# ZhiHuangHn/vtkCloudPoint

Measured on AMD Instinct MI355X. Metric: Mpoints/s DBSCAN+label @10M pts, higher is better.
Workload: dtype f64; 1 GPU; C4: 10000000-pt cloud (half uniform background, 200 Gaussian blobs), one monolithic DBImproved.dbscan, metric L1_2D, eps 0.1, minPts 10; mode=single, points_total=10000000, points_per_gpu=10000000, clusters=27380, resident_in_hbm=True

## Files before the change

vtkcloudpoint_amd/csrc/gridbuild.hip:

```cpp
#include <algorithm>
#include <mutex>
#include <unordered_map>

#include "grid_common.hpp"

using namespace vcpg;

namespace {

constexpr int PT = 1024;
constexpr int PCH_MIN = 8192;
constexpr int FT = 1024;
constexpr uint32_t MAXB = 8192;
constexpr uint32_t wcap(int) { return 4096u; }
constexpr uint32_t QUEUE_FROM = 32;

typedef float4 Rec;

template <int GD>
__device__ __forceinline__ Rec rec_make(const float* qf, uint32_t idx, uint32_t cell) {
  return GD == 2 ? make_float4(qf[0], qf[1], __uint_as_float(idx), __uint_as_float(cell))
                 : make_float4(qf[0], qf[1], qf[2], __uint_as_float(idx));
}
template <int GD>
__device__ __forceinline__ uint32_t rec_cell(const Rec& r, const GridP& g, uint32_t& idx) {
  if (GD == 2) {
    idx = __float_as_uint(r.z);
    return __float_as_uint(r.w);
  }
  idx = __float_as_uint(r.w);
  const float qf[3] = {r.x, r.y, r.z};
  int cc[3];
  return cell_of32<3>(qf, g, cc);
}

template <int GD>
__device__ __forceinline__ uint32_t point_cell(const double* __restrict__ c, int64_t i, int stride, const GridP& g, float* qf) {
  double q[3];
  int cc[3];
  load_in<GD>(c, i, stride, q);
#pragma unroll
  for (int a = 0; a < GD; a++) qf[a] = rel32(q[a], g.mn[a], g.scale);
  return cell_of32<GD>(qf, g, cc);
}

struct PartGeom {
  uint32_t csh;
  uint32_t B;
  uint32_t a;
  uint32_t NS;
  uint32_t chunk;
  uint32_t nchunk;
};

inline int env_int(const char* name, int dflt, int lo, int hi) {
  const char* e = getenv(name);
  int v = e ? atoi(e) : dflt;
  return v < lo ? lo : v > hi ? hi : v;
}

inline PartGeom part_geom(int64_t n, uint32_t ncells) {
  static const int csh_max = env_int("VCP_CPB_LOG2", 14, 10, 14);
  static const int target = env_int("VCP_PART_CHUNKS", 256, 64, 8192);
  PartGeom p;
  int csh = csh_max;
  while (csh > 10 && ((uint64_t)ncells >> csh) * 4096ull < (uint64_t)n) csh--;
  p.csh = (uint32_t)csh;
  p.B = (uint32_t)((((uint64_t)ncells + 1) + ((1ull << p.csh) - 1)) >> p.csh);
  p.a = 0;
  while (((p.B + (1u << p.a) - 1u) >> p.a) > MAXB) p.a++;
  p.NS = (p.B + (1u << p.a) - 1u) >> p.a;
  int64_t chunk = (n + target - 1) / target;
  if (chunk < PCH_MIN) chunk = PCH_MIN;
  chunk = (chunk + PT - 1) / PT * PT;
  p.chunk = (uint32_t)chunk;
  p.nchunk = (uint32_t)((n + chunk - 1) / chunk);
  return p;
}

template <int GD, bool GROUPED>
__global__ __launch_bounds__(PT) void k_part_hist(const double* __restrict__ c, int64_t n, int stride, GridP g,
                                                 const int32_t* __restrict__ group, int glo, int ghi, uint32_t csh,
                                                 uint32_t B, uint32_t chunk, uint32_t nchunk,
                                                 uint32_t* __restrict__ counts, uint32_t* __restrict__ qcount,
                                                 uint32_t* __restrict__ ctcount) {
  extern __shared__ uint32_t h[];
  if (blockIdx.x == 0 && threadIdx.x == 0) {
    *qcount = 0u;
    ctcount[0] = 0u;
  }
  for (uint32_t k = threadIdx.x; k < B; k += PT) h[k] = 0;
  __syncthreads();
  const int64_t first = (int64_t)blockIdx.x * chunk;
  const int64_t last = min(first + (int64_t)chunk, n);
#pragma unroll 4
  for (int64_t i = first + threadIdx.x; i < last; i += PT) {
    if (GROUPED) {
      const int gg = group[i];
      if (gg < glo || gg >= ghi) continue;
    }
    float qf[3];
    atomicAdd(&h[point_cell<GD>(c, i, stride, g, qf) >> csh], 1u);
  }
  __syncthreads();
  for (uint32_t k = threadIdx.x; k < B; k += PT) counts[(size_t)k * nchunk + blockIdx.x] = h[k];
}

template <int GD, bool GROUPED>
__global__ __launch_bounds__(PT) void k_part_scatter(const double* __restrict__ c, int64_t n, int stride, GridP g,
                                                    const int32_t* __restrict__ group, int glo, int ghi, uint32_t csh,
                                                    uint32_t B, uint32_t chunk, uint32_t nchunk,
                                                    const uint32_t* __restrict__ base, Rec* __restrict__ rec,
                                                    uint32_t* __restrict__ pos) {
  extern __shared__ uint32_t h[];
  for (uint32_t k = threadIdx.x; k < B; k += PT) h[k] = base[(size_t)k * nchunk + blockIdx.x];
  __syncthreads();
  const int64_t first = (int64_t)blockIdx.x * chunk;
  const int64_t last = min(first + (int64_t)chunk, n);
#pragma unroll 4
  for (int64_t i = first + threadIdx.x; i < last; i += PT) {
    if (GROUPED) {
      const int gg = group[i];
      if (gg < glo || gg >= ghi) {
        if (pos) pos[i] = NONE;
        continue;
      }
    }
    float qf[3];
    const uint32_t cell = point_cell<GD>(c, i, stride, g, qf);
    rec[atomicAdd(&h[cell >> csh], 1u)] = rec_make<GD>(qf, (uint32_t)i, cell);
  }
}

__device__ __forceinline__ uint32_t padded(uint32_t i) { return i + (i >> 5); }

template <int GD, bool GROUPED, int NT = FT>
__device__ __forceinline__ void fine_flush(uint32_t s0, uint32_t m, const float* s32, const uint32_t* sidx,
                                           const uint32_t* __restrict__ ord, const uint8_t* __restrict__ in_classed,
                                           const int32_t* __restrict__ group, float* __restrict__ sorted32,
                                           uint32_t* __restrict__ sord, uint32_t* __restrict__ sidx_out,
                                           int32_t* __restrict__ sgroup, uint8_t* __restrict__ flags,
                                           uint32_t* __restrict__ pos) {
  if (GD == 2) {
    const float2* src = reinterpret_cast<const float2*>(s32);
    float2* dst = reinterpret_cast<float2*>(sorted32) + s0;
    for (uint32_t k = threadIdx.x; k < m; k += NT) dst[k] = src[k];
  } else {
    const float4* src = reinterpret_cast<const float4*>(s32);
    float4* dst = reinterpret_cast<float4*>(sorted32) + s0;
    for (uint32_t k = threadIdx.x; k < m; k += NT) dst[k] = src[k];
  }
  for (uint32_t k = threadIdx.x; k < m; k += NT) {
    const uint32_t i = sidx[k], p = s0 + k;
    sord[p] = ord ? ord[i] : i;
    if (sidx_out) sidx_out[p] = i;
    if (GROUPED) sgroup[p] = group[i];
    if (in_classed) flags[p] = in_classed[i] ? F_CLASSED : 0;
    if (pos) pos[i] = p;
  }
}

template <int GD>
__device__ __forceinline__ void stage_put(float* s32, uint32_t* sidx, uint32_t p, const Rec& r, uint32_t idx) {
  if (GD == 2) reinterpret_cast<float2*>(s32)[p] = make_float2(r.x, r.y);
  else reinterpret_cast<float4*>(s32)[p] = make_float4(r.x, r.y, r.z, 0.0f);
  sidx[p] = idx;
}

__device__ __forceinline__ void bucket_range(const uint32_t* __restrict__ bstart, uint32_t bstride, const uint32_t* __restrict__ total,
                                             uint32_t b, uint32_t B, uint32_t& s, uint32_t& e) {
  s = bstart[(size_t)b * bstride];
  e = (b + 1 < B) ? bstart[(size_t)(b + 1) * bstride] : *total;
}

template <int GD>
__global__ __launch_bounds__(FT) void k_part_split(const Rec* __restrict__ rec, Rec* __restrict__ rec2,
                                                  const uint32_t* __restrict__ base, const uint32_t* __restrict__ total,
                                                  uint32_t nchunk, uint32_t NS, uint32_t a, uint32_t csh, uint32_t B, GridP g,
                                                  uint32_t* __restrict__ bstart) {
  __shared__ uint32_t h[32];
  const uint32_t S = blockIdx.x;
  uint32_t s, e;
  bucket_range(base, nchunk, total, S, NS, s, e);
  const uint32_t subm = (1u << a) - 1u;
  if (threadIdx.x < 32) h[threadIdx.x] = 0u;
  __syncthreads();
  for (uint32_t j = s + threadIdx.x; j < e; j += FT) {
    uint32_t i;
    atomicAdd(&h[(rec_cell<GD>(rec[j], g, i) >> csh) & subm], 1u);
  }
  __syncthreads();
  if (threadIdx.x < 32) {
    const uint32_t v = h[threadIdx.x];
    uint32_t inc = v;
#pragma unroll
    for (int d = 1; d < 32; d <<= 1) {
      const uint32_t t = __shfl_up(inc, d, 64);
      if ((int)threadIdx.x >= d) inc += t;
    }
    const uint32_t first = s + inc - v;
    h[threadIdx.x] = first;
    const uint32_t bk = (S << a) + threadIdx.x;
    if (threadIdx.x <= subm && bk <= B) bstart[bk] = first;
  }
  __syncthreads();
  for (uint32_t j = s + threadIdx.x; j < e; j += FT) {
    const Rec r = rec[j];
    uint32_t i;
    rec2[atomicAdd(&h[(rec_cell<GD>(r, g, i) >> csh) & subm], 1u)] = r;
  }
}

constexpr int FS = 512;
constexpr uint32_t scap(int gd) { return gd == 2 ? 2048u : 1536u; }
constexpr uint32_t SPOP = 128;

template <int GD, bool GROUPED>
__global__ __launch_bounds__(FS) void k_part_fine_small(const Rec* __restrict__ rec, const uint32_t* __restrict__ bstart,
                                                       uint32_t bstride, const uint32_t* __restrict__ total, uint32_t B,
                                                       uint32_t csh, GridP g, const uint32_t* __restrict__ ord,
                                                       const uint8_t* __restrict__ in_classed, const int32_t* __restrict__ group,
                                                       uint4* __restrict__ ctwords, uint32_t* __restrict__ ctdense,
                                                       uint32_t* __restrict__ ctcount, uint8_t* __restrict__ bstate,
                                                       float* __restrict__ sorted32, uint32_t* __restrict__ sord,
                                                       uint32_t* __restrict__ sidx_out, int32_t* __restrict__ sgroup,
                                                       uint8_t* __restrict__ flags, uint32_t* __restrict__ pos) {
  constexpr uint32_t FPR = GD == 2 ? 2 : 4;
  constexpr uint32_t SCAP = scap(GD);
  constexpr int SRPT = SCAP / FS;
  __shared__ uint32_t ws[512 + 2];
  __shared__ uint32_t wlo[512], whi[512];
  __shared__ uint16_t wpi[512];
  __shared__ uint8_t sci[SCAP];
  __shared__ __attribute__((aligned(16))) uint16_t st32[SPOP][32];
  __shared__ __attribute__((aligned(16))) float s32[SCAP * FPR];
  __shared__ uint32_t sidx[SCAP];
  __shared__ uint32_t wsum[FS / 64];
  __shared__ uint32_t s_np, s_dbase;
  const uint32_t b = blockIdx.x;
  uint32_t s, e;
  bucket_range(bstart, bstride, total, b, B, s, e);
  const uint32_t m = e - s;
  if (b + 1 == B && threadIdx.x == 0) ctcount[1] = *total;
  if (m > SCAP) {
    if (threadIdx.x == 0) bstate[b] = 1;
    return;
  }
  const uint32_t CPB = 1u << csh, NW = CPB >> 5, c0 = b << csh;
  const int lane = threadIdx.x & 63, w = threadIdx.x >> 6;
  for (uint32_t k = threadIdx.x; k < NW + 1; k += FS) ws[k] = 0u;
  __syncthreads();
  Rec r[SRPT];
  uint32_t idx[SRPT], lw[SRPT], ci[SRPT], rnk[SRPT];
#pragma unroll
  for (int k = 0; k < SRPT; k++) {
    const uint32_t j = s + (uint32_t)k * FS + threadIdx.x;
    lw[k] = NONE;
    if (j < e) {
      r[k] = rec[j];
      const uint32_t c = rec_cell<GD>(r[k], g, idx[k]) - c0;
      lw[k] = c >> 5;
      ci[k] = c & 31u;
      rnk[k] = atomicAdd(&ws[lw[k]], 1u);
    }
  }
  __syncthreads();
  {
    const uint32_t v = threadIdx.x < NW ? ws[threadIdx.x] : 0u;
    uint32_t inc = v;
#pragma unroll
    for (int d = 1; d < 64; d <<= 1) {
      const uint32_t t = __shfl_up(inc, d, 64);
      if (lane >= d) inc += t;
    }
    if (lane == 63) wsum[w] = inc;
    __syncthreads();
    uint32_t pre = inc - v;
    for (int k = 0; k < w; k++) pre += wsum[k];
    if (threadIdx.x < NW) ws[threadIdx.x] = s + pre;
    if (threadIdx.x == 0) ws[NW] = e;
  }
  __syncthreads();
#pragma unroll
  for (int k = 0; k < SRPT; k++)
    if (lw[k] != NONE) sci[ws[lw[k]] - s + rnk[k]] = (uint8_t)ci[k];
  __syncthreads();
  bool popl = false;
  uint32_t lo = 0u, hi = 0u;
  if (threadIdx.x < NW) {
    const uint32_t a = ws[threadIdx.x] - s, k = ws[threadIdx.x + 1] - s - a;
    if (k > 64u) {
      popl = true;
    } else {
      for (uint32_t i = 0; i < k; i++) {
        const uint32_t bit = 1u << sci[a + i];
        if (lo & hi & bit) continue;
        if (lo & bit) hi ^= bit;
        lo ^= bit;
      }
      popl = (lo & hi) != 0u;
    }
  }
  {
    const unsigned long long dm = __ballot(popl);
    if (lane == 0) wsum[w] = (uint32_t)__popcll(dm);
    __syncthreads();
    uint32_t before = (uint32_t)__popcll(dm & ((1ull << lane) - 1ull)), tot = 0;
    for (int k = 0; k < FS / 64; k++) {
      if (k < w) before += wsum[k];
      tot += wsum[k];
    }
    if (threadIdx.x == 0) s_np = tot;
    if (threadIdx.x < NW) wpi[threadIdx.x] = popl ? (uint16_t)before : (uint16_t)0xFFFFu;
  }
  __syncthreads();
  const uint32_t np = s_np;
  if (np > SPOP) {
    if (threadIdx.x == 0) bstate[b] = 1;
    return;
  }
  if (threadIdx.x == 0) {
    bstate[b] = 0;
    s_dbase = np ? atomicAdd(&ctcount[0], np) : 0u;
  }
  for (uint32_t k = threadIdx.x; k < np * 16u; k += FS) reinterpret_cast<uint32_t*>(&st32[0][0])[k] = 0u;
  if (threadIdx.x < NW && !popl) {
    wlo[threadIdx.x] = lo;
    whi[threadIdx.x] = hi;
  }
  __syncthreads();
#pragma unroll
  for (int k = 0; k < SRPT; k++)
    if (lw[k] != NONE && wpi[lw[k]] != 0xFFFFu) {
      uint16_t* c = &st32[wpi[lw[k]]][ci[k]];
      atomicAdd(reinterpret_cast<uint32_t*>(reinterpret_cast<uintptr_t>(c) & ~(uintptr_t)3), ((uintptr_t)c & 2) ? 0x10000u : 1u);
    }
  __syncthreads();
  {
    const uint32_t hw = threadIdx.x >> 5, li = threadIdx.x & 31u;
    for (uint32_t wd = hw; wd < NW; wd += FS / 32) {
      const uint32_t pi = wpi[wd];
      if (pi == 0xFFFFu) continue;
      const uint32_t c = st32[pi][li];
      uint32_t inc = c;
#pragma unroll
      for (int d = 1; d < 32; d <<= 1) {
        const uint32_t t = __shfl_up(inc, d, 32);
        if ((int)li >= d) inc += t;
      }
      const uint32_t first = ws[wd] + inc - c;
      st32[pi][li] = (uint16_t)(first - s);
      ctdense[(size_t)(s_dbase + pi) * 32u + li] = first;
      const uint32_t cs = min(c, 3u);
      const unsigned long long blo = __ballot(cs & 1u), bhi = __ballot(cs >> 1);
      const int sh = (threadIdx.x & 32) ? 32 : 0;
      if (li == 0) {
        wlo[wd] = (uint32_t)(blo >> sh);
        whi[wd] = (uint32_t)(bhi >> sh);
      }
    }
  }
  __syncthreads();
#pragma unroll
  for (int k = 0; k < SRPT; k++) {
    if (lw[k] == NONE) continue;
    const uint32_t pi = wpi[lw[k]];
    uint32_t p;
    if (pi != 0xFFFFu) {
      uint16_t* c = &st32[pi][ci[k]];
      const bool up = ((uintptr_t)c & 2) != 0;
      const uint32_t old = atomicAdd(reinterpret_cast<uint32_t*>(reinterpret_cast<uintptr_t>(c) & ~(uintptr_t)3), up ? 0x10000u : 1u);
      p = up ? old >> 16 : old & 0xFFFFu;
    } else {
      const uint32_t l = wlo[lw[k]], h = whi[lw[k]], below = (1u << ci[k]) - 1u;
      const uint32_t a = ws[lw[k]] - s;
      p = a + (uint32_t)__popc(l & below) + 2u * (uint32_t)__popc(h & below);
      if ((h >> ci[k]) & 1u)
        for (uint32_t i = 0; i < rnk[k]; i++) p += sci[a + i] == (uint8_t)ci[k] ? 1u : 0u;
    }
    stage_put<GD>(s32, sidx, p, r[k], idx[k]);
  }
  if (threadIdx.x < NW) {
    const size_t W = (size_t)(c0 >> 5) + threadIdx.x;
    const uint32_t pi = wpi[threadIdx.x];
    if (W < vcp_ct_words(g.ncells))
      ctwords[W] = make_uint4(wlo[threadIdx.x], whi[threadIdx.x], ws[threadIdx.x], pi != 0xFFFFu ? s_dbase + pi : NONE);
  }
  __syncthreads();
  fine_flush<GD, GROUPED, FS>(s, m, s32, sidx, ord, in_classed, group, sorted32, sord, sidx_out, sgroup, flags, pos);
}

template <int GD, bool GROUPED>
__global__ __launch_bounds__(FT) void k_part_fine(const Rec* __restrict__ rec, uint32_t* __restrict__ rk,
                                                 const uint32_t* __restrict__ bstart, uint32_t bstride,
                                                 const uint32_t* __restrict__ total, uint32_t B, uint32_t csh, GridP g,
                                                 const uint32_t* __restrict__ ord, const uint8_t* __restrict__ in_classed,
                                                 const int32_t* __restrict__ group, uint4* __restrict__ ctwords,
                                                 uint32_t* __restrict__ ctdense, uint32_t* __restrict__ ctcount,
                                                 float* __restrict__ sorted32, uint32_t* __restrict__ sord,
                                                 uint32_t* __restrict__ sidx_out, int32_t* __restrict__ sgroup,
                                                 uint8_t* __restrict__ flags, uint32_t* __restrict__ pos,
                                                 uint2* __restrict__ queue, uint32_t* __restrict__ qcount,
                                                 const uint8_t* __restrict__ bstate) {
  extern __shared__ __attribute__((aligned(16))) unsigned char lds[];
  __shared__ uint32_t wsum[FT / 64];
  __shared__ uint32_t w_lo[512], w_hi[512], w_slot[512];
  __shared__ uint32_t s_dbase;
  const uint32_t b = blockIdx.x;
  if (bstate[b] == 0) return;
  constexpr uint32_t WCAP = wcap(GD);
  constexpr uint32_t FPR = GD == 2 ? 2 : 4;
  const uint32_t CPB = 1u << csh;
  uint32_t* cnt = reinterpret_cast<uint32_t*>(lds);
  float* s32 = reinterpret_cast<float*>(lds + (((size_t)padded(CPB) + 4) & ~3ull) * 4);
  uint32_t* sidx = reinterpret_cast<uint32_t*>(s32 + (size_t)WCAP * FPR);
  const uint32_t c0 = b << csh;
  uint32_t s, e;
  bucket_range(bstart, bstride, total, b, B, s, e);
  const uint32_t m = e - s;
  const bool big = m > WCAP;
  for (uint32_t k = threadIdx.x; k < padded(CPB); k += FT) cnt[k] = 0;
  __syncthreads();
  for (uint32_t j = s + threadIdx.x; j < e; j += FT) {
    uint32_t i;
    uint32_t* slot = &cnt[padded(rec_cell<GD>(rec[j], g, i) - c0)];
    if (big) rk[j] = atomicAdd(slot, 1u);
    else atomicAdd(slot, 1u);
  }
  __syncthreads();
  const uint32_t PER = CPB / FT;
  const uint32_t first = threadIdx.x * PER;
  uint32_t loc = 0;
  for (uint32_t k = 0; k < PER; k++) loc += cnt[padded(first + k)];
  const int lane = threadIdx.x & 63, w = threadIdx.x >> 6;
  uint32_t inc = loc;
#pragma unroll
  for (int d = 1; d < 64; d <<= 1) {
    const uint32_t t = __shfl_up(inc, d, 64);
    if (lane >= d) inc += t;
  }
  if (lane == 63) wsum[w] = inc;
  __syncthreads();
  uint32_t pre = s + inc - loc;
  for (int k = 0; k < w; k++) pre += wsum[k];
  const uint32_t NW = CPB >> 5;
  uint32_t plo = 0u, phi = 0u;
  const uint32_t wstart = pre;
  {
    const uint32_t bit0 = first & 31u;
    for (uint32_t k = 0; k < PER; k++) {
      const uint32_t v = cnt[padded(first + k)];
      cnt[padded(first + k)] = pre;
      pre += v;
      const uint32_t c = min(v, 3u);
      plo |= (c & 1u) << (bit0 + k);
      phi |= (c >> 1) << (bit0 + k);
    }
    for (uint32_t d = 1; d < 32u / PER; d <<= 1) {
      plo |= (uint32_t)__shfl_xor((int)plo, (int)d, 64);
      phi |= (uint32_t)__shfl_xor((int)phi, (int)d, 64);
    }
    if ((first & 31u) == 0u) {
      w_lo[first >> 5] = plo;
      w_hi[first >> 5] = phi;
      w_slot[first >> 5] = wstart;
    }
  }
  __syncthreads();
  {
    const bool popl = threadIdx.x < NW && (w_lo[threadIdx.x] & w_hi[threadIdx.x]) != 0u;
    const unsigned long long dm = __ballot(popl);
    if (lane == 0) wsum[w] = (uint32_t)__popcll(dm);
    __syncthreads();
    uint32_t before = (uint32_t)__popcll(dm & ((1ull << lane) - 1ull)), tot = 0;
    for (int k = 0; k < FT / 64; k++) {
      if (k < w) before += wsum[k];
      tot += wsum[k];
    }
    if (threadIdx.x == 0) s_dbase = tot ? atomicAdd(&ctcount[0], tot) : 0u;
    __syncthreads();
    if (threadIdx.x < NW) {
      const uint32_t slot = popl ? s_dbase + before : NONE;
      const uint32_t wpos = w_slot[threadIdx.x];
      w_slot[threadIdx.x] = slot;
      const size_t W = (size_t)(c0 >> 5) + threadIdx.x;
      if (W < vcp_ct_words(g.ncells))
        ctwords[W] = make_uint4(w_lo[threadIdx.x], w_hi[threadIdx.x], wpos, slot);
    }
    __syncthreads();
    const uint32_t hw = threadIdx.x >> 5, li = threadIdx.x & 31u;
    for (uint32_t j = hw; j < NW; j += FT / 32) {
      const uint32_t slot = w_slot[j];
      if (slot != NONE) ctdense[(size_t)slot * 32u + li] = cnt[padded(32u * j + li)];
    }
  }
  __syncthreads();
  if (!big) {
    for (uint32_t j = s + threadIdx.x; j < e; j += FT) {
      const Rec r = rec[j];
      uint32_t i;
      const uint32_t p = atomicAdd(&cnt[padded(rec_cell<GD>(r, g, i) - c0)], 1u) - s;
      stage_put<GD>(s32, sidx, p, r, i);
    }
    __syncthreads();
    fine_flush<GD, GROUPED>(s, m, s32, sidx, ord, in_classed, group, sorted32, sord, sidx_out, sgroup, flags, pos);
    return;
  }
  if (m > QUEUE_FROM * WCAP) {
    __shared__ uint32_t q0;
    const uint32_t nwin = (m + WCAP - 1) / WCAP;
    if (threadIdx.x == 0) q0 = atomicAdd(qcount, nwin);
    __syncthreads();
    for (uint32_t k = threadIdx.x; k < nwin; k += FT) queue[q0 + k] = make_uint2(b, k * WCAP);
    return;
  }
  for (uint32_t w0 = 0; w0 < m; w0 += WCAP) {
    for (uint32_t j = s + threadIdx.x; j < e; j += FT) {
      const Rec r = rec[j];
      uint32_t i;
      const uint32_t p = cnt[padded(rec_cell<GD>(r, g, i) - c0)] + rk[j] - s - w0;
      if (p < WCAP) stage_put<GD>(s32, sidx, p, r, i);
    }
    __syncthreads();
    fine_flush<GD, GROUPED>(s + w0, min(WCAP, m - w0), s32, sidx, ord, in_classed, group, sorted32, sord, sidx_out, sgroup,
                            flags, pos);
    __syncthreads();
  }
}

template <int GD, bool GROUPED>
__global__ __launch_bounds__(FT) void k_part_fine_windows(const Rec* __restrict__ rec, const uint32_t* __restrict__ rk,
                                                         const uint32_t* __restrict__ bstart, uint32_t bstride,
                                                         const uint32_t* __restrict__ total, uint32_t B, GridP g,
                                                         const uint32_t* __restrict__ ord, const uint8_t* __restrict__ in_classed,
                                                         const int32_t* __restrict__ group, CellTab ct,
                                                         float* __restrict__ sorted32,
                                                         uint32_t* __restrict__ sord, uint32_t* __restrict__ sidx_out,
                                                         int32_t* __restrict__ sgroup, uint8_t* __restrict__ flags,
                                                         uint32_t* __restrict__ pos, const uint2* __restrict__ queue,
                                                         const uint32_t* __restrict__ qcount) {
  extern __shared__ __attribute__((aligned(16))) unsigned char lds[];
  constexpr uint32_t WCAP = wcap(GD);
  constexpr uint32_t FPR = GD == 2 ? 2 : 4;
  float* s32 = reinterpret_cast<float*>(lds);
  uint32_t* sidx = reinterpret_cast<uint32_t*>(s32 + (size_t)WCAP * FPR);
  const uint32_t nq = *qcount;
  for (uint32_t qi = blockIdx.x; qi < nq; qi += gridDim.x) {
    const uint2 q = queue[qi];
    const uint32_t b = q.x, w0 = q.y;
    uint32_t s, e;
    bucket_range(bstart, bstride, total, b, B, s, e);
    const uint32_t m = e - s;
    for (uint32_t j = s + threadIdx.x; j < e; j += FT) {
      const Rec r = rec[j];
      uint32_t i;
      const uint32_t p = ct_start(ct, rec_cell<GD>(r, g, i)) + rk[j] - s - w0;
      if (p < WCAP) stage_put<GD>(s32, sidx, p, r, i);
    }
    __syncthreads();
    fine_flush<GD, GROUPED>(s + w0, min(WCAP, m - w0), s32, sidx, ord, in_classed, group, sorted32, sord, sidx_out, sgroup,
                            flags, pos);
    __syncthreads();
  }
}

constexpr int OT = 1024, OPT = 16;
constexpr int OWT = 512;

template <int OWSH>
__global__ __launch_bounds__(OT) void k_out_scatter(const uint32_t* __restrict__ sord, const uint32_t* __restrict__ labk,
                                                   int64_t n, uint32_t OB, uint32_t* __restrict__ gcur,
                                                   uint2* __restrict__ rec) {
  extern __shared__ uint32_t h[];
  for (uint32_t k = threadIdx.x; k < OB; k += OT) h[k] = 0;
  __syncthreads();
  const int64_t first = (int64_t)blockIdx.x * (OT * OPT);
  uint32_t o[OPT], w[OPT], r[OPT];
#pragma unroll
  for (int k = 0; k < OPT; k++) {
    const int64_t p = first + (int64_t)k * OT + threadIdx.x;
    o[k] = NONE;
    if (p < n) {
      o[k] = sord[p];
      w[k] = labk[p];
      r[k] = atomicAdd(&h[o[k] >> OWSH], 1u);
    }
  }
  __syncthreads();
  for (uint32_t k = threadIdx.x; k < OB; k += OT) {
    const uint32_t c = h[k];
    if (c) h[k] = atomicAdd(&gcur[k], c);
  }
  __syncthreads();
#pragma unroll
  for (int k = 0; k < OPT; k++) {
    if (o[k] == NONE) continue;
    const uint32_t bk = o[k] >> OWSH;
    rec[((size_t)bk << OWSH) + h[bk] + r[k]] = make_uint2(o[k], w[k]);
  }
}

template <int OWSH>
__global__ __launch_bounds__(OWT) void k_out_write(const uint2* __restrict__ rec, int64_t n, bool have_in_classed,
                                                  int32_t cf_in, int32_t* __restrict__ labels,
                                                  uint8_t* __restrict__ is_core, uint8_t* __restrict__ is_classed,
                                                  unsigned long long* __restrict__ counters, uint32_t* __restrict__ gcur) {
  extern __shared__ __attribute__((aligned(16))) uint32_t sw[];
  if (threadIdx.x == 0) gcur[blockIdx.x] = 0u;
  const int64_t lo = (int64_t)blockIdx.x << OWSH;
  const uint32_t cnt = (uint32_t)min((int64_t)1 << OWSH, n - lo);
  unsigned unclassed = 0;
  for (uint32_t j = threadIdx.x; j < cnt; j += OWT) {
    const uint2 v = rec[lo + j];
    sw[v.x - (uint32_t)lo] = v.y;
    if (!(v.y & 2u)) unclassed++;
  }
  __syncthreads();
  auto lab_of = [&](uint32_t w) { return (w >> 2) ? cf_in + (int32_t)(w >> 2) : 0; };
  auto core_of = [](uint32_t w) { return (uint32_t)((w & 3u) == 1u); };
  auto cls_of = [](uint32_t w) { return (uint32_t)((w & 2u) != 0u || (w >> 2) != 0u); };
  const bool vec = (((uintptr_t)labels & 15u) | ((uintptr_t)is_core & 3u) | ((uintptr_t)is_classed & 3u)) == 0;
  const uint32_t c4 = vec ? cnt >> 2 : 0u;
  for (uint32_t j = threadIdx.x; j < c4; j += OWT) {
    const uint4 w = reinterpret_cast<const uint4*>(sw)[j];
    const int4 l = make_int4(lab_of(w.x), lab_of(w.y), lab_of(w.z), lab_of(w.w));
    if (have_in_classed) {
      if (l.x) labels[lo + 4 * j] = l.x;
      if (l.y) labels[lo + 4 * j + 1] = l.y;
      if (l.z) labels[lo + 4 * j + 2] = l.z;
      if (l.w) labels[lo + 4 * j + 3] = l.w;
    } else {
      reinterpret_cast<int4*>(labels + lo)[j] = l;
    }
    if (is_core)
      reinterpret_cast<uint32_t*>(is_core + lo)[j] = core_of(w.x) | core_of(w.y) << 8 | core_of(w.z) << 16 | core_of(w.w) << 24;
    if (is_classed)
      reinterpret_cast<uint32_t*>(is_classed + lo)[j] = cls_of(w.x) | cls_of(w.y) << 8 | cls_of(w.z) << 16 | cls_of(w.w) << 24;
  }
  for (uint32_t j = (c4 << 2) + threadIdx.x; j < cnt; j += OWT) {
    const uint32_t w = sw[j];
    const int32_t l = lab_of(w);
    if (!have_in_classed || l) labels[lo + j] = l;
    if (is_core) is_core[lo + j] = (uint8_t)core_of(w);
    if (is_classed) is_classed[lo + j] = (uint8_t)cls_of(w);
  }
  if (have_in_classed) {
    __shared__ unsigned wc[OWT / 64];
#pragma unroll
    for (int d = 32; d > 0; d >>= 1) unclassed += __shfl_down(unclassed, d, 64);
    if ((threadIdx.x & 63) == 0) wc[threadIdx.x >> 6] = unclassed;
    __syncthreads();
    if (threadIdx.x == 0) {
      unsigned t = 0;
      for (int k = 0; k < OWT / 64; k++) t += wc[k];
      if (t) atomicAdd(&counters[CNT_UNCLASSED + (blockIdx.x & (CNT_SPREAD - 1))], (unsigned long long)t);
    }
  }
}

int allow_lds(vcp_ctx* ctx, const void* kernel, size_t bytes) {
  static std::mutex mu;
  static std::unordered_map<uint64_t, size_t> allowed;
  std::lock_guard<std::mutex> lk(mu);
  const uint64_t key = (uint64_t)reinterpret_cast<uintptr_t>(kernel) * 64u + (uint64_t)(ctx->device & 63);
  size_t& have = allowed.emplace(key, (size_t)64 * 1024).first->second;
  if (bytes > have) {
    VCP_HIP(ctx, hipFuncSetAttribute(kernel, hipFuncAttributeMaxDynamicSharedMemorySize, (int)bytes));
    have = bytes;
  }
  return VCP_OK;
}
template <class K>
int allow_lds(vcp_ctx* ctx, K kernel, size_t bytes) {
  return allow_lds(ctx, reinterpret_cast<const void*>(kernel), bytes);
}

template <int GD, bool GROUPED>
int build(vcp_ctx* ctx, const GridBuildArgs& a) {
  hipStream_t st = ctx->stream;
  const PartGeom pg = part_geom(a.n, a.g.ncells);
  const size_t nc = (size_t)pg.NS * pg.nchunk;
  VCP_TRY(vcp_ensure(ctx, ctx->b_hist, (nc + 8) * 4));
  VCP_TRY(vcp_ensure(ctx, ctx->b_rec, (size_t)a.n * sizeof(Rec)));
  uint32_t* counts = ctx->b_hist.as<uint32_t>();
  uint32_t* total = counts + nc;
  Rec* rec = ctx->b_rec.as<Rec>();
  const size_t lds_h = (size_t)pg.NS * 4;
  const uint32_t CPB = 1u << pg.csh;
  const size_t lds_f = ((((size_t)CPB + CPB / 32) + 4) & ~3ull) * 4 + (size_t)wcap(GD) * ((GD == 2 ? 8 : 16) + 4);
  VCP_TRY(allow_lds(ctx, k_part_fine<GD, GROUPED>, lds_f));
  VCP_TRY(vcp_ensure(ctx, ctx->b_fineq, ((size_t)a.n / wcap(GD) + pg.B + 8) * sizeof(uint2) + 64));
  uint32_t* qcount = ctx->b_fineq.as<uint32_t>();
  uint2* queue = reinterpret_cast<uint2*>(ctx->b_fineq.as<char>() + 64);
  vcp_phase(ctx, "part_hist");
  const uint32_t csh_a = pg.csh + pg.a;
  VCP_LAUNCH(ctx, (k_part_hist<GD, GROUPED>), dim3(pg.nchunk), dim3(PT), lds_h, st, a.d_coords, a.n, a.stride, a.g,
                  a.d_group, a.glo, a.ghi, csh_a, pg.NS, pg.chunk, pg.nchunk, counts, qcount, a.ctcount);
  VCP_TRY(vcp_exclusive_scan_u32(ctx, counts, counts, (int64_t)nc, total));
  vcp_phase(ctx, "part_scatter");
  VCP_LAUNCH(ctx, (k_part_scatter<GD, GROUPED>), dim3(pg.nchunk), dim3(PT), lds_h, st, a.d_coords, a.n, a.stride, a.g,
                  a.d_group, a.glo, a.ghi, csh_a, pg.NS, pg.chunk, pg.nchunk, counts, rec, a.pos);
  const uint32_t* bstart = counts;
  uint32_t bstride = pg.nchunk;
  if (pg.a > 0) {
    vcp_phase(ctx, "part_split");
    VCP_TRY(vcp_ensure(ctx, ctx->b_rec2, (size_t)a.n * sizeof(Rec)));
    VCP_TRY(vcp_ensure(ctx, ctx->b_bstart, ((size_t)pg.B + 2) * 4));
    VCP_LAUNCH(ctx, k_part_split<GD>, dim3(pg.NS), dim3(FT), 0, st, rec, ctx->b_rec2.as<Rec>(), counts, total, pg.nchunk,
                    pg.NS, pg.a, pg.csh, pg.B, a.g, ctx->b_bstart.as<uint32_t>());
    rec = ctx->b_rec2.as<Rec>();
    bstart = ctx->b_bstart.as<uint32_t>();
    bstride = 1;
  }
  vcp_phase(ctx, "part_fine");
  VCP_TRY(vcp_ensure(ctx, ctx->b_rank, (size_t)a.n * 4));
  VCP_TRY(vcp_ensure(ctx, ctx->b_bstate, (size_t)pg.B + 16));
  uint8_t* bstate = ctx->b_bstate.as<uint8_t>();
  VCP_LAUNCH(ctx, (k_part_fine_small<GD, GROUPED>), dim3(pg.B), dim3(FS), 0, st, rec, bstart, bstride, total, pg.B, pg.csh,
                  a.g, a.d_ord, a.d_in_classed, a.d_group, a.ctwords, a.ctdense, a.ctcount, bstate, a.sorted32, a.sord,
                  a.sidx, a.sgroup, a.flags, a.pos);
  VCP_LAUNCH(ctx, (k_part_fine<GD, GROUPED>), dim3(pg.B), dim3(FT), lds_f, st, rec, ctx->b_rank.as<uint32_t>(), bstart,
                  bstride, total, pg.B, pg.csh, a.g, a.d_ord, a.d_in_classed, a.d_group, a.ctwords, a.ctdense, a.ctcount,
                  a.sorted32, a.sord, a.sidx, a.sgroup, a.flags, a.pos, queue, qcount, bstate);
  {
    const size_t lds_w = (size_t)wcap(GD) * ((GD == 2 ? 8 : 16) + 4);
    VCP_TRY(allow_lds(ctx, k_part_fine_windows<GD, GROUPED>, lds_w));
    const unsigned gw = (unsigned)std::min<size_t>(768, (size_t)a.n / wcap(GD) + 1);
    const CellTab ct{a.ctwords, a.ctdense, a.ctcount + 1};
    VCP_LAUNCH(ctx, (k_part_fine_windows<GD, GROUPED>), dim3(gw), dim3(FT), lds_w, st, rec, ctx->b_rank.as<uint32_t>(),
                    bstart, bstride, total, pg.B, a.g, a.d_ord, a.d_in_classed, a.d_group, ct, a.sorted32,
                    a.sord, a.sidx, a.sgroup, a.flags, a.pos, queue, qcount);
  }
  return VCP_OK;
}

}

int vcp_grid_build_partition(vcp_ctx* ctx, const GridBuildArgs& a) {
  const bool grouped = a.d_group != nullptr;
  if (a.gd == 3) {
    if (grouped) return vcp_fail(ctx, VCP_ERR_ARG, "grouped calls are 2-D");
    return build<3, false>(ctx, a);
  }
  return grouped ? build<2, true>(ctx, a) : build<2, false>(ctx, a);
}

template <int OWSH>
static int output_partition(vcp_ctx* ctx, const GridOutputArgs& a) {
  hipStream_t st = ctx->stream;
  const uint32_t OB = (uint32_t)((a.n + (1 << OWSH) - 1) >> OWSH);
  const void* before = ctx->b_outcur.p;
  const size_t before_cap = ctx->b_outcur.cap;
  VCP_TRY(vcp_ensure(ctx, ctx->b_outcur, ((size_t)OB + 8) * 4));
  if (ctx->b_outcur.p != before || ctx->b_outcur.cap != before_cap)
    VCP_HIP(ctx, hipMemsetAsync(ctx->b_outcur.p, 0, ctx->b_outcur.cap, st));
  VCP_TRY(vcp_ensure(ctx, ctx->b_rec, (size_t)OB << (OWSH + 3)));
  uint32_t* gcur = ctx->b_outcur.as<uint32_t>();
  uint2* rec = ctx->b_rec.as<uint2>();
  VCP_TRY(allow_lds(ctx, k_out_write<OWSH>, (size_t)4 << OWSH));
  vcp_phase(ctx, "out_scatter");
  VCP_LAUNCH(ctx, k_out_scatter<OWSH>, dim3(vcp_blocks(a.n, OT * OPT)), dim3(OT), (size_t)OB * 4, st, a.sord, a.labk, a.n,
                  OB, gcur, rec);
  vcp_phase(ctx, "out_write");
  VCP_LAUNCH(ctx, k_out_write<OWSH>, dim3(OB), dim3(OWT), (size_t)4 << OWSH, st, rec, a.n, a.have_in_classed, a.cf_in,
                  a.labels, a.is_core, a.is_classed, a.counters, gcur);
  return VCP_OK;
}

int vcp_grid_output_partition(vcp_ctx* ctx, const GridOutputArgs& a) {
  if (a.n > ((int64_t)1 << 27)) return vcp_fail(ctx, VCP_ERR_TOO_LARGE, "more than 2^27 points: use the gather output");
  if (a.n >= ((int64_t)1 << 23)) return output_partition<15>(ctx, a);
  if (a.n >= ((int64_t)1 << 22)) return output_partition<14>(ctx, a);
  return output_partition<13>(ctx, a);
}
```

Baseline: 7030 Mpoints/s.

## Add packed 16-bit cell counters and register-cached records to fine partition

Splits the fine partition kernel into a templated helper with two paths. Buckets of up to cap1 points (8192 in 2D) take a new PACKED path: two cell counters share one 32-bit LDS word, which halves the counter footprint so a larger staging window fits. Each thread loads its records once into registers and reuses them for both the histogram and scatter passes, instead of re-reading global memory and spilling to the rk rank buffer. The aim is to keep mid-size buckets off the multi-window or queued path and to cut global reads. The cost is higher register pressure and an LDS requirement sized for the larger of the two layouts, which may lower occupancy.

```diff
diff --git a/vtkcloudpoint_amd/csrc/gridbuild.hip b/vtkcloudpoint_amd/csrc/gridbuild.hip
--- a/vtkcloudpoint_amd/csrc/gridbuild.hip
+++ b/vtkcloudpoint_amd/csrc/gridbuild.hip
@@ -12,6 +12,7 @@
 constexpr int PCH_MIN = 8192;
 constexpr int FT = 1024;
 constexpr uint32_t MAXB = 8192;
+constexpr uint32_t cap1(int gd) { return gd == 2 ? 8192u : 6144u; }
 constexpr uint32_t wcap(int) { return 4096u; }
 constexpr uint32_t QUEUE_FROM = 32;
 
@@ -390,6 +391,181 @@
   fine_flush<GD, GROUPED, FS>(s, m, s32, sidx, ord, in_classed, group, sorted32, sord, sidx_out, sgroup, flags, pos);
 }
 
+struct FineSh {
+  uint32_t wsum[FT / 64];
+  uint32_t w_lo[512], w_hi[512], w_slot[512];
+  uint32_t s_dbase, q0;
+};
+
+template <int GD, bool GROUPED, bool PACKED>
+__device__ __forceinline__ void fine_bucket(FineSh& sh, unsigned char* lds, uint32_t b, uint32_t s, uint32_t e,
+                                            const Rec* __restrict__ rec, uint32_t* __restrict__ rk, uint32_t csh,
+                                            const GridP& g, const uint32_t* __restrict__ ord,
+                                            const uint8_t* __restrict__ in_classed, const int32_t* __restrict__ group,
+                                            uint4* __restrict__ ctwords, uint32_t* __restrict__ ctdense,
+                                            uint32_t* __restrict__ ctcount, float* __restrict__ sorted32,
+                                            uint32_t* __restrict__ sord, uint32_t* __restrict__ sidx_out,
+                                            int32_t* __restrict__ sgroup, uint8_t* __restrict__ flags,
+                                            uint32_t* __restrict__ pos, uint2* __restrict__ queue,
+                                            uint32_t* __restrict__ qcount) {
+  constexpr uint32_t WCAP = wcap(GD);
+  constexpr uint32_t SCAPF = PACKED ? cap1(GD) : WCAP;
+  constexpr uint32_t FPR = GD == 2 ? 2 : 4;
+  constexpr int RPT = cap1(GD) / FT;
+  const uint32_t CPB = 1u << csh;
+  const uint32_t NCW = PACKED ? CPB >> 1 : CPB;
+  uint32_t* cnt = reinterpret_cast<uint32_t*>(lds);
+  float* s32 = reinterpret_cast<float*>(lds + (((size_t)padded(NCW) + 4) & ~3ull) * 4);
+  uint32_t* sidx = reinterpret_cast<uint32_t*>(s32 + (size_t)SCAPF * FPR);
+  const uint32_t c0 = b << csh;
+  const uint32_t m = e - s;
+  for (uint32_t k = threadIdx.x; k < padded(NCW); k += FT) cnt[k] = 0;
+  __syncthreads();
+  Rec r[RPT];
+  uint32_t cc[RPT];
+  if (PACKED) {
+#pragma unroll
+    for (int k = 0; k < RPT; k++) {
+      const uint32_t j = s + (uint32_t)k * FT + threadIdx.x;
+      cc[k] = NONE;
+      if (j < e) {
+        r[k] = rec[j];
+        uint32_t i;
+        cc[k] = rec_cell<GD>(r[k], g, i) - c0;
+        atomicAdd(&cnt[padded(cc[k] >> 1)], 1u << (16u * (cc[k] & 1u)));
+      }
+    }
+  } else {
+    for (uint32_t j = s + threadIdx.x; j < e; j += FT) {
+      uint32_t i;
+      rk[j] = atomicAdd(&cnt[padded(rec_cell<GD>(rec[j], g, i) - c0)], 1u);
+    }
+  }
+  __syncthreads();
+  const uint32_t PER = PACKED ? max(2u, CPB / FT) : CPB / FT;
+  const uint32_t first = threadIdx.x * PER;
+  const bool own = first < CPB;
+  uint32_t loc = 0;
+  if (PACKED) {
+    if (own)
+      for (uint32_t k = 0; k < PER / 2; k++) {
+        const uint32_t v = cnt[padded((first >> 1) + k)];
+        loc += (v & 0xFFFFu) + (v >> 16);
+      }
+  } else {
+    for (uint32_t k = 0; k < PER; k++) loc += cnt[padded(first + k)];
+  }
+  const int lane = threadIdx.x & 63, w = threadIdx.x >> 6;
+  uint32_t inc = loc;
+#pragma unroll
+  for (int d = 1; d < 64; d <<= 1) {
+    const uint32_t t = __shfl_up(inc, d, 64);
+    if (lane >= d) inc += t;
+  }
+  if (lane == 63) sh.wsum[w] = inc;
+  __syncthreads();
+  uint32_t pre = (PACKED ? 0u : s) + inc - loc;
+  for (int k = 0; k < w; k++) pre += sh.wsum[k];
+  const uint32_t NW = CPB >> 5;
+  uint32_t plo = 0u, phi = 0u;
+  const uint32_t wstart = (PACKED ? s : 0u) + pre;
+  {
+    const uint32_t bit0 = first & 31u;
+    if (PACKED) {
+      if (own)
+        for (uint32_t k = 0; k < PER / 2; k++) {
+          const uint32_t at = padded((first >> 1) + k);
+          const uint32_t v = cnt[at], v0 = v & 0xFFFFu, v1 = v >> 16;
+          cnt[at] = pre | (pre + v0) << 16;
+          pre += v0 + v1;
+          const uint32_t a0 = min(v0, 3u), a1 = min(v1, 3u);
+          plo |= ((a0 & 1u) | (a1 & 1u) << 1) << (bit0 + 2u * k);
+          phi |= ((a0 >> 1) | (a1 >> 1) << 1) << (bit0 + 2u * k);
+        }
+    } else {
+      for (uint32_t k = 0; k < PER; k++) {
+        const uint32_t v = cnt[padded(first + k)];
+        cnt[padded(first + k)] = pre;
+        pre += v;
+        const uint32_t c = min(v, 3u);
+        plo |= (c & 1u) << (bit0 + k);
+        phi |= (c >> 1) << (bit0 + k);
+      }
+    }
+    for (uint32_t d = 1; d < 32u / PER; d <<= 1) {
+      plo |= (uint32_t)__shfl_xor((int)plo, (int)d, 64);
+      phi |= (uint32_t)__shfl_xor((int)phi, (int)d, 64);
+    }
+    if (own && (first & 31u) == 0u) {
+      sh.w_lo[first >> 5] = plo;
+      sh.w_hi[first >> 5] = phi;
+      sh.w_slot[first >> 5] = wstart;
+    }
+  }
+  __syncthreads();
+  {
+    const bool popl = threadIdx.x < NW && (sh.w_lo[threadIdx.x] & sh.w_hi[threadIdx.x]) != 0u;
+    const unsigned long long dm = __ballot(popl);
+    if (lane == 0) sh.wsum[w] = (uint32_t)__popcll(dm);
+    __syncthreads();
+    uint32_t before = (uint32_t)__popcll(dm & ((1ull << lane) - 1ull)), tot = 0;
+    for (int k = 0; k < FT / 64; k++) {
+      if (k < w) before += sh.wsum[k];
+      tot += sh.wsum[k];
+    }
+    if (threadIdx.x == 0) sh.s_dbase = tot ? atomicAdd(&ctcount[0], tot) : 0u;
+    __syncthreads();
+    if (threadIdx.x < NW) {
+      const uint32_t slot = popl ? sh.s_dbase + before : NONE;
+      const uint32_t wpos = sh.w_slot[threadIdx.x];
+      sh.w_slot[threadIdx.x] = slot;
+      const size_t W = (size_t)(c0 >> 5) + threadIdx.x;
+      if (W < vcp_ct_words(g.ncells))
+        ctwords[W] = make_uint4(sh.w_lo[threadIdx.x], sh.w_hi[threadIdx.x], wpos, slot);
+    }
+    __syncthreads();
+    const uint32_t hw = threadIdx.x >> 5, li = threadIdx.x & 31u;
+    for (uint32_t j = hw; j < NW; j += FT / 32) {
+      const uint32_t slot = sh.w_slot[j];
+      if (slot == NONE) continue;
+      if (PACKED) ctdense[(size_t)slot * 32u + li] = s + ((cnt[padded(16u * j + (li >> 1))] >> (16u * (li & 1u))) & 0xFFFFu);
+      else ctdense[(size_t)slot * 32u + li] = cnt[padded(32u * j + li)];
+    }
+  }
+  __syncthreads();
+  if (PACKED) {
+#pragma unroll
+    for (int k = 0; k < RPT; k++) {
+      if (cc[k] == NONE) continue;
+      const uint32_t sft = 16u * (cc[k] & 1u);
+      const uint32_t p = (atomicAdd(&cnt[padded(cc[k] >> 1)], 1u << sft) >> sft) & 0xFFFFu;
+      stage_put<GD>(s32, sidx, p, r[k], __float_as_uint(GD == 2 ? r[k].z : r[k].w));
+    }
+    __syncthreads();
+    fine_flush<GD, GROUPED>(s, m, s32, sidx, ord, in_classed, group, sorted32, sord, sidx_out, sgroup, flags, pos);
+    return;
+  }
+  if (m > QUEUE_FROM * WCAP) {
+    const uint32_t nwin = (m + WCAP - 1) / WCAP;
+    if (threadIdx.x == 0) sh.q0 = atomicAdd(qcount, nwin);
+    __syncthreads();
+    for (uint32_t k = threadIdx.x; k < nwin; k += FT) queue[sh.q0 + k] = make_uint2(b, k * WCAP);
+    return;
+  }
+  for (uint32_t w0 = 0; w0 < m; w0 += WCAP) {
+    for (uint32_t j = s + threadIdx.x; j < e; j += FT) {
+      const Rec r1 = rec[j];
+      uint32_t i;
+      const uint32_t p = cnt[padded(rec_cell<GD>(r1, g, i) - c0)] + rk[j] - s - w0;
+      if (p < WCAP) stage_put<GD>(s32, sidx, p, r1, i);
+    }
+    __syncthreads();
+    fine_flush<GD, GROUPED>(s + w0, min(WCAP, m - w0), s32, sidx, ord, in_classed, group, sorted32, sord, sidx_out, sgroup,
+                            flags, pos);
+    __syncthreads();
+  }
+}
+
 template <int GD, bool GROUPED>
 __global__ __launch_bounds__(FT) void k_part_fine(const Rec* __restrict__ rec, uint32_t* __restrict__ rk,
                                                  const uint32_t* __restrict__ bstart, uint32_t bstride,
@@ -403,129 +579,17 @@
                                                  uint2* __restrict__ queue, uint32_t* __restrict__ qcount,
                                                  const uint8_t* __restrict__ bstate) {
   extern __shared__ __attribute__((aligned(16))) unsigned char lds[];
-  __shared__ uint32_t wsum[FT / 64];
-  __shared__ uint32_t w_lo[512], w_hi[512], w_slot[512];
-  __shared__ uint32_t s_dbase;
+  __shared__ FineSh sh;
   const uint32_t b = blockIdx.x;
   if (bstate[b] == 0) return;
-  constexpr uint32_t WCAP = wcap(GD);
-  constexpr uint32_t FPR = GD == 2 ? 2 : 4;
-  const uint32_t CPB = 1u << csh;
-  uint32_t* cnt = reinterpret_cast<uint32_t*>(lds);
-  float* s32 = reinterpret_cast<float*>(lds + (((size_t)padded(CPB) + 4) & ~3ull) * 4);
-  uint32_t* sidx = reinterpret_cast<uint32_t*>(s32 + (size_t)WCAP * FPR);
-  const uint32_t c0 = b << csh;
   uint32_t s, e;
   bucket_range(bstart, bstride, total, b, B, s, e);
-  const uint32_t m = e - s;
-  const bool big = m > WCAP;
-  for (uint32_t k = threadIdx.x; k < padded(CPB); k += FT) cnt[k] = 0;
-  __syncthreads();
-  for (uint32_t j = s + threadIdx.x; j < e; j += FT) {
-    uint32_t i;
-    uint32_t* slot = &cnt[padded(rec_cell<GD>(rec[j], g, i) - c0)];
-    if (big) rk[j] = atomicAdd(slot, 1u);
-    else atomicAdd(slot, 1u);
-  }
-  __syncthreads();
-  const uint32_t PER = CPB / FT;
-  const uint32_t first = threadIdx.x * PER;
-  uint32_t loc = 0;
-  for (uint32_t k = 0; k < PER; k++) loc += cnt[padded(first + k)];
-  const int lane = threadIdx.x & 63, w = threadIdx.x >> 6;
-  uint32_t inc = loc;
-#pragma unroll
-  for (int d = 1; d < 64; d <<= 1) {
-    const uint32_t t = __shfl_up(inc, d, 64);
-    if (lane >= d) inc += t;
-  }
-  if (lane == 63) wsum[w] = inc;
-  __syncthreads();
-  uint32_t pre = s + inc - loc;
-  for (int k = 0; k < w; k++) pre += wsum[k];
-  const uint32_t NW = CPB >> 5;
-  uint32_t plo = 0u, phi = 0u;
-  const uint32_t wstart = pre;
-  {
-    const uint32_t bit0 = first & 31u;
-    for (uint32_t k = 0; k < PER; k++) {
-      const uint32_t v = cnt[padded(first + k)];
-      cnt[padded(first + k)] = pre;
-      pre += v;
-      const uint32_t c = min(v, 3u);
-      plo |= (c & 1u) << (bit0 + k);
-      phi |= (c >> 1) << (bit0 + k);
-    }
-    for (uint32_t d = 1; d < 32u / PER; d <<= 1) {
-      plo |= (uint32_t)__shfl_xor((int)plo, (int)d, 64);
-      phi |= (uint32_t)__shfl_xor((int)phi, (int)d, 64);
-    }
-    if ((first & 31u) == 0u) {
-      w_lo[first >> 5] = plo;
-      w_hi[first >> 5] = phi;
-      w_slot[first >> 5] = wstart;
-    }
-  }
-  __syncthreads();
-  {
-    const bool popl = threadIdx.x < NW && (w_lo[threadIdx.x] & w_hi[threadIdx.x]) != 0u;
-    const unsigned long long dm = __ballot(popl);
-    if (lane == 0) wsum[w] = (uint32_t)__popcll(dm);
-    __syncthreads();
-    uint32_t before = (uint32_t)__popcll(dm & ((1ull << lane) - 1ull)), tot = 0;
-    for (int k = 0; k < FT / 64; k++) {
-      if (k < w) before += wsum[k];
-      tot += wsum[k];
-    }
-    if (threadIdx.x == 0) s_dbase = tot ? atomicAdd(&ctcount[0], tot) : 0u;
-    __syncthreads();
-    if (threadIdx.x < NW) {
-      const uint32_t slot = popl ? s_dbase + before : NONE;
-      const uint32_t wpos = w_slot[threadIdx.x];
-      w_slot[threadIdx.x] = slot;
-      const size_t W = (size_t)(c0 >> 5) + threadIdx.x;
-      if (W < vcp_ct_words(g.ncells))
-        ctwords[W] = make_uint4(w_lo[threadIdx.x], w_hi[threadIdx.x], wpos, slot);
-    }
-    __syncthreads();
-    const uint32_t hw = threadIdx.x >> 5, li = threadIdx.x & 31u;
-    for (uint32_t j = hw; j < NW; j += FT / 32) {
-      const uint32_t slot = w_slot[j];
-      if (slot != NONE) ctdense[(size_t)slot * 32u + li] = cnt[padded(32u * j + li)];
-    }
-  }
-  __syncthreads();
-  if (!big) {
-    for (uint32_t j = s + threadIdx.x; j < e; j += FT) {
-      const Rec r = rec[j];
-      uint32_t i;
-      const uint32_t p = atomicAdd(&cnt[padded(rec_cell<GD>(r, g, i) - c0)], 1u) - s;
-      stage_put<GD>(s32, sidx, p, r, i);
-    }
-    __syncthreads();
-    fine_flush<GD, GROUPED>(s, m, s32, sidx, ord, in_classed, group, sorted32, sord, sidx_out, sgroup, flags, pos);
-    return;
-  }
-  if (m > QUEUE_FROM * WCAP) {
-    __shared__ uint32_t q0;
-    const uint32_t nwin = (m + WCAP - 1) / WCAP;
-    if (threadIdx.x == 0) q0 = atomicAdd(qcount, nwin);
-    __syncthreads();
-    for (uint32_t k = threadIdx.x; k < nwin; k += FT) queue[q0 + k] = make_uint2(b, k * WCAP);
-    return;
-  }
-  for (uint32_t w0 = 0; w0 < m; w0 += WCAP) {
-    for (uint32_t j = s + threadIdx.x; j < e; j += FT) {
-      const Rec r = rec[j];
-      uint32_t i;
-      const uint32_t p = cnt[padded(rec_cell<GD>(r, g, i) - c0)] + rk[j] - s - w0;
-      if (p < WCAP) stage_put<GD>(s32, sidx, p, r, i);
-    }
-    __syncthreads();
-    fine_flush<GD, GROUPED>(s + w0, min(WCAP, m - w0), s32, sidx, ord, in_classed, group, sorted32, sord, sidx_out, sgroup,
-                            flags, pos);
-    __syncthreads();
-  }
+  if (e - s <= cap1(GD))
+    fine_bucket<GD, GROUPED, true>(sh, lds, b, s, e, rec, rk, csh, g, ord, in_classed, group, ctwords, ctdense, ctcount,
+                                   sorted32, sord, sidx_out, sgroup, flags, pos, queue, qcount);
+  else
+    fine_bucket<GD, GROUPED, false>(sh, lds, b, s, e, rec, rk, csh, g, ord, in_classed, group, ctwords, ctdense, ctcount,
+                                    sorted32, sord, sidx_out, sgroup, flags, pos, queue, qcount);
 }
 
 template <int GD, bool GROUPED>
@@ -687,7 +751,9 @@
   Rec* rec = ctx->b_rec.as<Rec>();
   const size_t lds_h = (size_t)pg.NS * 4;
   const uint32_t CPB = 1u << pg.csh;
-  const size_t lds_f = ((((size_t)CPB + CPB / 32) + 4) & ~3ull) * 4 + (size_t)wcap(GD) * ((GD == 2 ? 8 : 16) + 4);
+  const size_t rec_f = (GD == 2 ? 8 : 16) + 4;
+  const size_t lds_f = std::max(((((size_t)CPB / 2 + CPB / 64) + 4) & ~3ull) * 4 + (size_t)cap1(GD) * rec_f,
+                                ((((size_t)CPB + CPB / 32) + 4) & ~3ull) * 4 + (size_t)wcap(GD) * rec_f);
   VCP_TRY(allow_lds(ctx, k_part_fine<GD, GROUPED>, lds_f));
   VCP_TRY(vcp_ensure(ctx, ctx->b_fineq, ((size_t)a.n / wcap(GD) + pg.B + 8) * sizeof(uint2) + 64));
   uint32_t* qcount = ctx->b_fineq.as<uint32_t>();
```

Measured after the change: 7137 Mpoints/s, median of 6. +1.5%, better.
